# cs2mosa/Heterogeneous-MOE-for-Diffusion-models

Measured on AMD Instinct MI355X. Metric: denoise-steps/sec (fwd+bwd) on 4x32x32 latents, higher is better.
Workload: dtype bf16

## Files before the change

heterogeneous-moe-for-diffusion-models_amd/csrc/common.h:

```cpp
#pragma once
#include <hip/hip_runtime.h>
#include <stdint.h>

#define HDMOE_OK 0
#define HDMOE_EINVAL (-1)
#define HDMOE_EDTYPE (-2)
#define HDMOE_ELAUNCH (-3)

#define HDMOE_F32 0
#define HDMOE_BF16 1
#define HDMOE_F32S 2
#define HDMOE_F16 3

#define HDMOE_MAX_GROUPS 8
#define MP_SILU_DIV 0.596f

typedef __bf16 bf16;
typedef __attribute__((ext_vector_type(8))) __bf16 bf16x8;
typedef __attribute__((ext_vector_type(4))) __bf16 bf16x4;
typedef __attribute__((ext_vector_type(2))) __bf16 bf16x2;
typedef __attribute__((ext_vector_type(16))) float f32x16;
typedef __attribute__((ext_vector_type(4))) float f32x4;

#define DEVI __device__ __forceinline__
// ... 89 lines not shown
}
template <> DEVI void vload<float>(float* f, const float* p) {
  const float4 v = *reinterpret_cast<const float4*>(p);
  f[0] = v.x; f[1] = v.y; f[2] = v.z; f[3] = v.w;
}
template <typename T> DEVI void vstore(T* p, const float* f);
template <> DEVI void vstore<bf16>(bf16* p, const float* f) {
  bf16x8 v;
#pragma unroll
  for (int j = 0; j < 8; ++j) v[j] = (bf16)f[j];
  *reinterpret_cast<bf16x8*>(p) = v;
}
template <> DEVI void vstore<float>(float* p, const float* f) { *reinterpret_cast<float4*>(p) = make_float4(f[0], f[1], f[2], f[3]); }
static inline bool al16(const void* p) { return p == nullptr || ((uintptr_t)p & 15) == 0; }

static inline int hdmoe_launch_status() {
  return hipGetLastError() == hipSuccess ? HDMOE_OK : HDMOE_ELAUNCH;
}
static inline bool hdmoe_first_on_device(unsigned long long& mask) {
  int dev = 0;
  (void)hipGetDevice(&dev);
  const unsigned long long bit = 1ull << (dev & 63);
  if (mask & bit) return false;
  mask |= bit;
  return true;
}
static inline unsigned cdiv(long a, long b) { return (unsigned)((a + b - 1) / b); }

DEVI void philox(uint32_t c0, uint32_t c1, uint32_t k0, uint32_t k1, uint32_t* o) {
  uint32_t c[4] = {c0, c1, 0u, 0u};
// ... 19 lines not shown
```

heterogeneous-moe-for-diffusion-models_amd/csrc/elementwise.hip:

```cpp
#include "common.h"
#include "hdmoe.h"

namespace {

constexpr int TPB = 256;
static inline unsigned grid_for(long n) {
  long b = (n + TPB - 1) / TPB;
  if (b > 2048) b = 2048;
  if (b < 1) b = 1;
  return (unsigned)b;
}
#define GRID_STRIDE(i, n) for (long i = (long)blockIdx.x * blockDim.x + threadIdx.x; i < (n); i += (long)gridDim.x * blockDim.x)

template <typename T>
__global__ void axpby_kernel(T* out, const T* x, const T* y, float a, float b, long n) {
  GRID_STRIDE(i, n) {
    float v = a * to_f(x[i]);
    if (y) v += b * to_f(y[i]);
    out[i] = from_f<T>(v);
  }
}
template <typename T>
__global__ void affine_kernel(T* out, const T* x, float a, float c, long n) {
  GRID_STRIDE(i, n) out[i] = from_f<T>(a * to_f(x[i]) + c);
// ... 582 lines not shown
__global__ void nhwc_to_nchw_guided_kernel(float* out, const T* F, const float* sf, const float* x, const float* sx, float g, int C, long HW,
                                           long n) {
  const float gu = 1.f - g;
  GRID_STRIDE(i, n) {
    long t = i; const long p = t % HW; t /= HW;
    const int c = (int)(t % C); const long b = t / C;
    const long f = (b * HW + p) * C + c;
    float v = gu * to_f(F[n + f]) + g * to_f(F[f]);
    if (sf) v *= sf[b];
    if (x) v += (sx ? sx[b] : 1.f) * x[i];
    out[i] = v;
  }
}

template <typename T, bool TO_IMG>
__global__ void patch_relayout_kernel(T* out, const T* in, int H, int W, int C, int p, int hp, int wp, int order, long n) {
  GRID_STRIDE(i, n) {
    long t = i; const int c = (int)(t % C); t /= C;
    const int x = (int)(t % W); t /= W;
    const int y = (int)(t % H); const long b = t / H;
    const int ph = y / p, ii = y % p, pw = x / p, jj = x % p;
    const int f = order ? c * p * p + ii * p + jj : (ii * p + jj) * C + c;
    const long tk = ((b * hp + ph) * wp + pw) * ((long)C * p * p) + f;
    if (TO_IMG) out[i] = in[tk];
    else out[tk] = in[i];
  }
}

template <typename T, bool TO_IMG>
__global__ void patch_relayout_vec_kernel(T* out, const T* in, int H, int W, int C, int p, int hp, int wp, int order, long nv) {
  constexpr int VW = VT<T>::W;
  const int CV = C / VW;
  GRID_STRIDE(i, nv) {
    long t = i; const int c0 = (int)(t % CV) * VW; t /= CV;
    const int x = (int)(t % W); t /= W;
    const int y = (int)(t % H); const long b = t / H;
    const int ph = y / p, ii = y - ph * p, pw = x / p, jj = x - pw * p;
    const long tb = ((b * hp + ph) * wp + pw) * ((long)C * p * p);
    T* img = (TO_IMG ? out : const_cast<T*>(in)) + i * VW;
    if (order == 0) {
      T* tk = (TO_IMG ? const_cast<T*>(in) : out) + tb + (long)(ii * p + jj) * C + c0;
      if (TO_IMG) *reinterpret_cast<uint4*>(img) = *reinterpret_cast<const uint4*>(tk);
      else *reinterpret_cast<uint4*>(tk) = *reinterpret_cast<const uint4*>(img);
    } else {
      const int pp = p * p;
      T* tk = (TO_IMG ? const_cast<T*>(in) : out) + tb + (long)c0 * pp + ii * p + jj;
      alignas(16) T v[VW];
      if (TO_IMG) {
#pragma unroll
        for (int k = 0; k < VW; ++k) v[k] = tk[(long)k * pp];
        *reinterpret_cast<uint4*>(img) = *reinterpret_cast<const uint4*>(v);
      } else {
        *reinterpret_cast<uint4*>(v) = *reinterpret_cast<const uint4*>(img);
#pragma unroll
        for (int k = 0; k < VW; ++k) tk[(long)k * pp] = v[k];
      }
    }
  }
}

template <typename T>
__global__ void patch_to_tokens_o1_vec_kernel(T* tok, const T* img, int H, int W, int C, int p, int hp, int wp, long nv) {
  constexpr int VW = VT<T>::W;
  const int jv = p / VW;
  GRID_STRIDE(v, nv) {
    long t = v;
    const int j0 = (int)(t % jv) * VW; t /= jv;
    const int ii = (int)(t % p); t /= p;
    const int c = (int)(t % C); t /= C;
    const int pw = (int)(t % wp); t /= wp;
    const int ph = (int)(t % hp); const long b = t / hp;
    const int y = ph * p + ii, x0 = pw * p + j0;
    alignas(16) T vals[VW];
#pragma unroll
    for (int k = 0; k < VW; ++k) vals[k] = (y < H && x0 + k < W) ? img[((b * H + y) * W + x0 + k) * C + c] : from_f<T>(0.f);
    *reinterpret_cast<uint4*>(tok + v * VW) = *reinterpret_cast<const uint4*>(vals);
  }
}

__global__ void fourier_kernel(float* out, const float* x, const float* freqs, const float* phases, int F, long n) {
  GRID_STRIDE(i, n) {
    const long b = i / F; const int f = (int)(i - b * F);
    out[i] = cosf(x[b] * freqs[f] + phases[f]) * 1.41421356237309515f;
  }
}
__global__ void edm_coeffs_kernel(float* coef, const float* sigma, int nsig, float sd, int B) {
  GRID_STRIDE(b, B) {
    const float s = sigma[nsig == 1 ? 0 : b];
    const float q = s * s + sd * sd;
    coef[b] = sd * sd / q;
// ... 690 lines not shown
int hdmoe_nchw_to_nhwc(void* out, const float* x, const float* s, int N, int C, long HW, int dtype, hipStream_t stream) {
  const long n = (long)N * C * HW;
  DT_SWITCH(dtype, L1D(nchw_to_nhwc_kernel<T>, n, (T*)out, x, s, C, HW, n))
}
int hdmoe_nhwc_to_nchw(float* out, const void* F, const float* sf, const float* x, const float* sx, int N, int C, long HW,
                       int dtype, hipStream_t stream) {
  const long n = (long)N * C * HW;
  DT_SWITCH(dtype, L1D(nhwc_to_nchw_kernel<T>, n, out, (const T*)F, sf, x, sx, C, HW, n))
}
int hdmoe_nhwc_to_nchw_guided(float* out, const void* F, const float* sf, const float* x, const float* sx, float g, int N, int C, long HW,
                              int dtype, hipStream_t stream) {
  if (!out || !F || N < 1 || C < 1 || HW < 1 || !(g == g) || g - g != 0.f) return HDMOE_EINVAL;
  const long n = (long)N * C * HW;
  DT_SWITCH(dtype, L1D(nhwc_to_nchw_guided_kernel<T>, n, out, (const T*)F, sf, x, sx, g, C, HW, n))
}
int hdmoe_patch_relayout(void* out, const void* in, int N, int H, int W, int C, int p, int hp, int wp, int order,
                         int to_img, int dtype, hipStream_t stream) {
  if (hp * p < H || wp * p < W) return HDMOE_EINVAL;
  const long n = (long)N * H * W * C;
  if (!to_img && order == 1 && al16(out) && (dtype == HDMOE_BF16 || dtype == HDMOE_F32) && p % (dtype == HDMOE_BF16 ? 8 : 4) == 0) {
    const long nv = (long)N * hp * wp * C * p * p / (dtype == HDMOE_BF16 ? 8 : 4);
    DT_SWITCH(dtype, L1D(patch_to_tokens_o1_vec_kernel<T>, nv, (T*)out, (const T*)in, H, W, C, p, hp, wp, nv))
  }
  if (al16(out) && al16(in) && C % (dtype == HDMOE_BF16 ? 8 : 4) == 0 && (dtype == HDMOE_BF16 || dtype == HDMOE_F32)) {
    const long nv = n / (dtype == HDMOE_BF16 ? 8 : 4);
    if (to_img) { DT_SWITCH(dtype, L1D((patch_relayout_vec_kernel<T, true>), nv, (T*)out, (const T*)in, H, W, C, p, hp, wp, order, nv)) }
    else { DT_SWITCH(dtype, L1D((patch_relayout_vec_kernel<T, false>), nv, (T*)out, (const T*)in, H, W, C, p, hp, wp, order, nv)) }
  }
  if (to_img) { DT_SWITCH(dtype, L1D((patch_relayout_kernel<T, true>), n, (T*)out, (const T*)in, H, W, C, p, hp, wp, order, n)) }
  else { DT_SWITCH(dtype, L1D((patch_relayout_kernel<T, false>), n, (T*)out, (const T*)in, H, W, C, p, hp, wp, order, n)) }
}
int hdmoe_fourier(float* out, const float* x, const float* freqs, const float* phases, int B, int F, hipStream_t stream) {
  const long n = (long)B * F;
  L1D(fourier_kernel, n, out, x, freqs, phases, F, n);
  return hdmoe_launch_status();
}
int hdmoe_edm_coeffs(float* coef, const float* sigma, int nsig, float sigma_data, int B, hipStream_t stream) {
  if (nsig != 1 && nsig != B) return HDMOE_EINVAL;
  L1D(edm_coeffs_kernel, B, coef, sigma, nsig, sigma_data, B);
  return hdmoe_launch_status();
}
int hdmoe_sigmoid_scaling(float* sv, float* su, float* pair, const float* c_noise, float tp, float soft, int B,
                          hipStream_t stream) {
  L1D(sigmoid_scaling_kernel, B, sv, su, pair, c_noise, tp, soft, B);
  return hdmoe_launch_status();
// ... 35 lines not shown
```

heterogeneous-moe-for-diffusion-models_amd/csrc/relayout.hip:

```cpp
#include "common.h"
#include "conv_args.h"
#include "hdmoe.h"

namespace {

constexpr int TPB = 256;
constexpr int RL_MAXV = 8;
constexpr int RL_TILE_MAX = RL_MAXV * TPB * 16;
constexpr int RL_TILE_TARGET = RL_TILE_MAX / 2;
constexpr int RL_PMAX = 64;
constexpr int RL_LDS_BYTES = RL_TILE_MAX + RL_PMAX * 16;
constexpr int RL_GRID = 512;

struct RlArgs {
  void* tok; void* img;
  int H, W, C, p, hp, wp, TW, tpr;
  long ntiles;
};

struct RlTile {
  long img0, tok0;
  int nvec, rowv, RS;
  int ylim, xlimv;
};
template <typename T, int P>
DEVI RlTile rl_tile(const RlArgs& a, long t) {
  constexpr int VW = VT<T>::W;
  const int p = P ? P : a.p;
  const long band = t / a.tpr;
  const int pw0 = (int)(t - band * a.tpr) * a.TW;
  const int tw = a.wp - pw0 < a.TW ? a.wp - pw0 : a.TW;
  const long b = band / a.hp;
// ... 35 lines not shown
  constexpr int VW = VT<T>::W;
  const int p = P ? P : a.p;
  const int jvn = p / VW, KV = a.C * p * jvn;
  const int tl = v / KV, rem = v - tl * KV;
  const int jv = rem % jvn, t2 = rem / jvn;
  const int ii = t2 % p, c = t2 / p;
  return ii * g.RS + (tl * p + jv * VW) * a.C + c;
}

template <typename T, int P, bool TO_IMG>
__global__ __launch_bounds__(TPB) void patch_relayout_tiled_kernel(RlArgs a) {
  constexpr int VW = VT<T>::W;
  __shared__ uint4 lds4[RL_LDS_BYTES / 16];
  T* lds = reinterpret_cast<T*>(lds4);
  uint4 r[RL_MAXV];
  long t = blockIdx.x;
  if (t >= a.ntiles) return;
  RlTile g = rl_tile<T, P>(a, t);
  rl_load<T, P, TO_IMG>(r, a, g);
  while (true) {
#pragma unroll
    for (int k = 0; k < RL_MAXV; ++k) {
      const int v = (int)threadIdx.x + k * TPB;
      if (v < g.nvec) {
        if (TO_IMG) {
          const int o = rl_tok_lds<T, P>(a, g, v);
          alignas(16) T e[VW];
          *reinterpret_cast<uint4*>(e) = r[k];
#pragma unroll
          for (int j = 0; j < VW; ++j) lds[o + j * a.C] = e[j];
        } else {
          const int ii = v / g.rowv, rest = v - ii * g.rowv;
          *reinterpret_cast<uint4*>(lds + ii * g.RS + rest * VW) = r[k];
        }
      }
    }
    __syncthreads();
    const long tn = t + gridDim.x;
    const RlTile gc = g;
    if (tn < a.ntiles) {
      g = rl_tile<T, P>(a, tn);
      rl_load<T, P, TO_IMG>(r, a, g);
    }
#pragma unroll
    for (int k = 0; k < RL_MAXV; ++k) {
      const int v = (int)threadIdx.x + k * TPB;
      if (v < gc.nvec) {
        if (TO_IMG) {
          const int ii = v / gc.rowv, rest = v - ii * gc.rowv;
          if (ii < gc.ylim && rest < gc.xlimv)
            *reinterpret_cast<uint4*>(static_cast<T*>(a.img) + gc.img0 + (long)ii * a.W * a.C + (long)rest * VW) =
                *reinterpret_cast<const uint4*>(lds + ii * gc.RS + rest * VW);
        } else {
          const int o = rl_tok_lds<T, P>(a, gc, v);
          alignas(16) T e[VW];
#pragma unroll
          for (int j = 0; j < VW; ++j) e[j] = lds[o + j * a.C];
          *reinterpret_cast<uint4*>(static_cast<T*>(a.tok) + gc.tok0 + (long)v * VW) = *reinterpret_cast<const uint4*>(e);
        }
      }
    }
    if (tn >= a.ntiles) break;
    t = tn;
    __syncthreads();
  }
}

template <typename T, bool TO_IMG>
int rl_launch(const RlArgs& a, unsigned grid, hipStream_t stream) {
  constexpr int VW = VT<T>::W;
  if (a.p == VW) hipLaunchKernelGGL((patch_relayout_tiled_kernel<T, VW, TO_IMG>), dim3(grid), dim3(TPB), 0, stream, a);
  else if (a.p == 2 * VW) hipLaunchKernelGGL((patch_relayout_tiled_kernel<T, 2 * VW, TO_IMG>), dim3(grid), dim3(TPB), 0, stream, a);
  else if (a.p == 4 * VW) hipLaunchKernelGGL((patch_relayout_tiled_kernel<T, 4 * VW, TO_IMG>), dim3(grid), dim3(TPB), 0, stream, a);
  else hipLaunchKernelGGL((patch_relayout_tiled_kernel<T, 0, TO_IMG>), dim3(grid), dim3(TPB), 0, stream, a);
  return hdmoe_launch_status();
}

constexpr int CR_U = 4;

// ... 56 lines not shown
      vstore<T>(dys + r * L + i, o);
      if (dot) {
        float y[VW];
        vload<T>(y, ys + r * L + i);
#pragma unroll
        for (int k = 0; k < VW; ++k) acc += g[k] * y[k];
      }
    }
  }
  if (dsparse) {
    acc = block_sum(acc, sm);
    if (threadIdx.x == 0 && b >= 0) atomicAdd(&dsparse[(long)b * E + row_expert[r]], acc);
  }
}

}

extern "C" {

int hdmoe_patch_relayout_tiled(void* out, const void* in, int N, int H, int W, int C, int p, int hp, int wp, int order, int to_img,
                               int dtype, hipStream_t stream) {
  if (!out || !in || N < 0 || H < 1 || W < 1 || C < 1 || p < 1 || hp < 1 || wp < 1 || (long)hp * p < H || (long)wp * p < W) return HDMOE_EINVAL;
  if (order != 1 || (dtype != HDMOE_BF16 && dtype != HDMOE_F32)) return 1;
  const int VW = dtype == HDMOE_BF16 ? 8 : 4, esz = dtype == HDMOE_BF16 ? 2 : 4;
  if (p % VW || C % VW || p > RL_PMAX || !al16(out) || !al16(in)) return 1;
  const long tokb = (long)C * p * p * esz;
  if (tokb > RL_TILE_MAX) return 1;
  if (N == 0) return HDMOE_OK;
  RlArgs a;
  a.tok = to_img ? const_cast<void*>(in) : out;
  a.img = to_img ? out : const_cast<void*>(in);
  a.H = H; a.W = W; a.C = C; a.p = p; a.hp = hp; a.wp = wp;
  long TW = RL_TILE_TARGET / tokb;
  if (TW < 1) TW = 1;
  if (TW > wp) TW = wp;
  a.TW = (int)TW;
  a.tpr = (wp + a.TW - 1) / a.TW;
  a.ntiles = (long)N * hp * a.tpr;
  if ((long)N * hp * wp * (tokb / esz) >= (1l << 40)) return 1;
  const unsigned grid = (unsigned)(a.ntiles < RL_GRID ? a.ntiles : RL_GRID);
  hdmoe_count_selection(HDMOE_SEL_RELAYOUT_TILED);
  if (dtype == HDMOE_BF16) return to_img ? rl_launch<bf16, true>(a, grid, stream) : rl_launch<bf16, false>(a, grid, stream);
  return to_img ? rl_launch<float, true>(a, grid, stream) : rl_launch<float, false>(a, grid, stream);
}

int hdmoe_combine_rows_fwd_vec(void* out, const void* ys, const int* inv, const float* row_w, long B, int kcap, long L, int dtype,
                               hipStream_t stream) {
  if (dtype != HDMOE_F32 && dtype != HDMOE_BF16) return HDMOE_EDTYPE;
  if (!out || !ys || !inv || B < 0 || kcap < 1 || L < 1) return HDMOE_EINVAL;
  const int VW = dtype == HDMOE_BF16 ? 8 : 4;
  if (L % VW || !al16(out) || !al16(ys)) return 1;
  if (B == 0) return HDMOE_OK;
  const long nck = cdiv(L, (long)TPB * CR_U * VW);
  if (B * nck >= (1l << 31)) return 1;
  hdmoe_count_selection(HDMOE_SEL_COMBINE_FWD_VEC);
  if (dtype == HDMOE_F32) hipLaunchKernelGGL(combine_rows_fwd_vec_kernel<float>, dim3((unsigned)(B * nck)), dim3(TPB), 0, stream, (float*)out, (const float*)ys, inv, row_w, kcap, L, (unsigned)nck);
  else hipLaunchKernelGGL(combine_rows_fwd_vec_kernel<bf16>, dim3((unsigned)(B * nck)), dim3(TPB), 0, stream, (bf16*)out, (const bf16*)ys, inv, row_w, kcap, L, (unsigned)nck);
  return hdmoe_launch_status();
// ... 18 lines not shown
```

heterogeneous-moe-for-diffusion-models_amd/hdmoe_hip/ops.py:

```python
from __future__ import annotations

import ctypes
import math
from typing import List, Optional, Sequence

import torch

from . import bank as _bank
from ._lib import dtype_code_cast
from ._lib import _int_array, call, dtype_code, lib

Tensor = torch.Tensor


def _c(t: Optional[Tensor]) -> Optional[Tensor]:
    if t is None:
        return None
    return t if t.is_contiguous() else t.contiguous()


def _dt(t: Tensor) -> int:
    return dtype_code(t.dtype)


# ... 651 lines not shown
        ents = [bank.lookup(ws, torch.float32, float(gain), 1.0, True) for ws in layers]
        ok = all(e is not None for e in ents) and len({(e.I, e.Ipad, len(e.params)) for e in ents if e is not None}) == 1
        if ok and all(e.khs == [1] * len(e.params) for e in ents) and (seg is not None or len(ents[0].params) == 1):
            flat = [w for ws in layers for w in ws]
            return list(_MultiLinearFn.apply(x, seg, ents, bank, float(c), *flat))
    outs = [mp_conv(x, ws if seg is not None else ws[0], gain, seg=seg, training=training) for ws in layers]
    return [affine(o, 1.0, c) for o in outs] if c != 0.0 else outs



def _call_or(fast: str, plain: str, *args) -> None:
    if call(fast, *args) == 1:
        call(plain, *args)


class _PatchLinearFn(torch.autograd.Function):

    @staticmethod
    def forward(ctx, x, w, b):
        x = _c(x)
        N, H, W, C = x.shape
        E, p = int(w.shape[0]), int(w.shape[2])
        hp, wp, K = H // p, W // p, C * p * p
        Epad = (E + 15) // 16 * 16
        tok = torch.empty((N, hp, wp, K), dtype=x.dtype, device=x.device)
        _call_or("hdmoe_patch_relayout_tiled", "hdmoe_patch_relayout", tok, x, N, H, W, C, p, hp, wp, 1, 0, _dt(x))
        wf = torch.empty(E * K, dtype=x.dtype, device=x.device)
        wd = torch.empty(K * Epad, dtype=x.dtype, device=x.device) if ctx.needs_input_grad[0] else None
        call("hdmoe_wprep_fwd", [w], None, 1.0, [1], [1], 1, E, K, K, Epad, wf, wf.numel(), wd, 0 if wd is None else wd.numel(), 0, 0, 0, _dt(x))
        y0 = torch.empty((N, hp, wp, E), dtype=x.dtype, device=x.device)
# ... 3 lines not shown
        ctx.save_for_backward(tok, w)
        ctx.wd = wd
        ctx.dims = (N, H, W, C, E, p, hp, wp, K, Epad)
        return y.reshape(N, hp * wp, E)

    @staticmethod
    def backward(ctx, dy):
        tok, w = ctx.saved_tensors
        N, H, W, C, E, p, hp, wp, K, Epad = ctx.dims
        dy = _c(dy).reshape(N, hp, wp, E)
        dt = _dt(dy)
        dx = dw = db = None
        if ctx.needs_input_grad[0]:
            dtok = torch.empty((N, hp, wp, K), dtype=dy.dtype, device=dy.device)
            call("hdmoe_conv_fwd", dy, ctx.wd, dtok, None, 1.0, 0.0, None, 1, ctx.wd.numel(), N, hp, wp, hp, wp, E, E, Epad, K, K, 1, 0, [1], [1], [0], [0], dt)
            dx = torch.empty((N, H, W, C), dtype=dy.dtype, device=dy.device)
            _call_or("hdmoe_patch_relayout_tiled", "hdmoe_patch_relayout", dx, dtok, N, H, W, C, p, hp, wp, 1, 1, dt)
        if ctx.needs_input_grad[1]:
            Gs = [_zeros((1, E, K), torch.float32, dy.device)]
            call("hdmoe_conv_wgrad", tok, dy, Gs, None, 1, N, hp, wp, hp, wp, K, K, E, 1, 0, [1], [1], [0], [0], dt)
            dw = torch.empty_like(w)
            call("hdmoe_wprep_bwd", [w], None, 1.0, Gs, [dw], None, [1], [1], 1, E, K, 0)
        if ctx.needs_input_grad[2]:
            db = torch.zeros(E, dtype=torch.float32, device=dy.device)
            call("hdmoe_colsum", db, dy, N * hp * wp, E, dt)
        return dx, dw, db


class _PatchEmbedFn(torch.autograd.Function):

    @staticmethod
    def forward(ctx, x, w, b):
# ... 17 lines not shown
        x, w = ctx.saved_tensors
        N, H, W, C = x.shape
        E, p = int(w.shape[0]), int(w.shape[2])
        hp, wp = -(-H // p), -(-W // p)
        dy = _c(dy).reshape(N, hp, wp, E)
        dx = dw = db = None
        if ctx.needs_input_grad[0]:
            Ipad = (C + 15) // 16 * 16
            Epad = (E + 15) // 16 * 16
            wf = torch.empty(p * p * E * Ipad, dtype=x.dtype, device=x.device)
            wd = torch.empty(p * p * C * Epad, dtype=x.dtype, device=x.device)
            call("hdmoe_wprep_fwd", [w], None, 1.0, [p], [p], 1, E, C, Ipad, Epad, wf, wf.numel(), wd, wd.numel(), 0, 0, 0, _dt(x))
            tok = torch.empty((N, hp, wp, p * p * C), dtype=x.dtype, device=x.device)
            call("hdmoe_conv_fwd", dy, wd, tok, None, 1.0, 0.0, None, 1, wd.numel(), N, hp, wp, hp, wp, E, E, Epad, p * p * C,
                 p * p * C, 1, 0, [1], [1], [0], [0], _dt(x))
            dx = torch.empty_like(x)
            call("hdmoe_patch_relayout", dx, tok, N, H, W, C, p, hp, wp, 0, 1, _dt(x))
        if ctx.needs_input_grad[1]:
            Gs = [_zeros((p * p, E, C), torch.float32, x.device)]
            call("hdmoe_conv_wgrad", x, dy, Gs, None, 1, N, H, W, hp, wp, C, C, E, p, 0, [p], [p], [0], [0], _dt(x))
            dw = torch.empty_like(w)
            call("hdmoe_wprep_bwd", [w], None, 1.0, Gs, [dw], None, [p], [p], 1, E, C, 0)
        if ctx.needs_input_grad[2]:
            db = torch.zeros(E, dtype=torch.float32, device=x.device)
            call("hdmoe_colsum", db, dy, N * hp * wp, E, _dt(x))
        return dx, dw, db


def patch_embed(x: Tensor, w: Tensor, b: Tensor) -> Tensor:
    p = int(w.shape[2])
    if (x.shape[1] % p == 0 and x.shape[2] % p == 0 and w.shape[2] == w.shape[3] and w.is_contiguous()
            and x.shape[3] % (8 if x.dtype == torch.bfloat16 else 4) == 0 and (x.shape[3] * p * p) % 16 == 0):
        return _PatchLinearFn.apply(x, w, b)
    return _PatchEmbedFn.apply(x, w, b)


class _AxpbyFn(torch.autograd.Function):
    @staticmethod
    def forward(ctx, x, y, a, b):
        x = _c(x); y = _c(y)
        out = torch.empty_like(x)
        call("hdmoe_axpby", out, x, y, a, b, x.numel(), _dt(x))
        ctx.ab = (a, b, y is not None)
        return out

    @staticmethod
    def backward(ctx, g):
        a, b, has_y = ctx.ab
        g = _c(g)
# ... 885 lines not shown

    @staticmethod
    def backward(ctx, g):
        N, H, W, C, p, hp, wp, order = ctx.meta
        g = _c(g)
        dtok = torch.zeros(ctx.tshape, dtype=g.dtype, device=g.device) if (hp * p != H or wp * p != W) else \
            torch.empty(ctx.tshape, dtype=g.dtype, device=g.device)
        _call_or("hdmoe_patch_relayout_tiled", "hdmoe_patch_relayout", dtok, g, N, H, W, C, p, hp, wp, order, 0, _dt(g))
        return dtok, None


def pixel_shuffle_tokens(tok: Tensor, H: int, W: int, C: int, p: int) -> Tensor:
    N = tok.shape[0]
    hp, wp = -(-H // p), -(-W // p)
    return _PatchRelayoutFn.apply(tok, (N, H, W, C, p, hp, wp, 1))


class _PixelNormFn(torch.autograd.Function):
    @staticmethod
    def forward(ctx, x, with_silu, gx_scale=1.0):
        ctx.sx = float(gx_scale)
        x = _c(x)
        C = x.shape[-1]
        xn = torch.empty_like(x)
        h = torch.empty_like(x) if with_silu else None
        call("hdmoe_pixelnorm_fwd", xn, h, x, x.numel() // C, C, _dt(x))
        ctx.save_for_backward(x)
        ctx.with_silu = with_silu
        if with_silu:
            return xn, h
# ... 661 lines not shown
```

heterogeneous-moe-for-diffusion-models_amd/models/model_components.py:

```python
from __future__ import annotations

from typing import List, Optional, Sequence

import torch
import torch.nn as nn

import models.model_internals as m
from hdmoe_hip import ops

Tensor = torch.Tensor


class Scaling_router(nn.Module):

    def __init__(self, emb_dim: Optional[int] = 3, num_experts: Optional[int] = 2, dropout: Optional[float] = 0.2):
        super().__init__()
        self.soft_route = nn.Sequential(
            m.MP_Conv(in_channels=emb_dim, out_channels=emb_dim * 2, kernel=()),
            nn.GroupNorm(1, emb_dim * 2),
            nn.ReLU(),
            m.MP_Conv(in_channels=emb_dim * 2, out_channels=emb_dim * 4, kernel=()),
            nn.GroupNorm(1, emb_dim * 4),
            nn.ReLU(),
            nn.Dropout(dropout),
# ... 424 lines not shown
    h = ops.ln_rag(yn, [b.norm2.weight for b in blocks], [b.norm2.bias for b in blocks], rag, b0.norm2.eps)
    h = ops.mp_silu(lin([b.linear2 for b in blocks], h, b0.gain_s))
    h = lin([b.linear3 for b in blocks], h, b0.gain_s, res=y, alpha=(1.0 - bal) / n, beta=bal / n, res_grad_raw=True)
    if b0.skip_proj is not None:
        return lin([b.skip_proj for b in blocks], res_main, b0.gain_s, res=h, alpha=(1.0 - bal) / n, beta=bal / n)
    return ops.mp_sum(res_main, h, bal)


def vit_expert_bank_forward(experts: Sequence["Vit_expert"], x: Tensor, time_emb: Optional[Tensor], text_emb: Optional[Tensor],
                            seg: Tensor) -> Tensor:
    e0 = experts[0]
    tr = e0.training
    R, H, W, C = x.shape
    ps = [e.patch.kernel_size[0] for e in experts]
    rag = ops.RagLayout(seg, [(-(-H // p)) * (-(-W // p)) for p in ps], R)
    pes = [ops.patch_embed(xe, e.patch.weight, e.patch.bias) for xe, e in zip(ops.fanout(x, len(experts)), experts)]
    tok = ops.rag_pack(pes, [e.pos_emb for e in experts], rag)
    t = time_emb
    if text_emb is not None:
        tx = text_emb
        if e0.map_txt is not None:
            tx = ops.mp_conv(tx, [e.map_txt.weights for e in experts], seg=seg, training=tr)
        t = ops.mp_sum(t, tx, e0.emb_balance)
    nb = len(e0.diffit)
    timed = t is not None and e0.diffit[0].TMSA.time_dependent
    tps = ts = None
    if timed and 3 * nb <= 16 and len({b.gain_t for b in e0.diffit}) == 1:
        layers = [[getattr(e.diffit[i].TMSA, nm).weights for e in experts] for i in range(nb) for nm in ("q_time", "k_time", "v_time")]
        tps = ops.multi_linear(t, layers, e0.diffit[0].gain_t, seg=seg, training=tr)
    elif timed:
        ts = list(ops.fanout(t, 3 * nb))
    for i in range(nb):
        tok = vit_block_bank_forward([e.diffit[i] for e in experts], tok, t if ts is None else ts[3 * i:3 * i + 3], rag,
                                     None if tps is None else tps[3 * i:3 * i + 3])
    tok = ops.ln_rag(tok, [e.norm.weight for e in experts], [e.norm.bias for e in experts], rag, e0.norm.eps)
    outs = []
    for e, p, part in zip(experts, ps, ops.rag_unpack(tok, rag)):
        outs.append(ops.pixel_shuffle_tokens(e.unpatch_proj._fwd(part), H, W, C, p))
    return ops.rag_select(outs, rag)
```

include/hdmoe.h:

```cpp
#ifndef HDMOE_H
#define HDMOE_H
#ifdef __cplusplus
extern "C" {
#endif

#ifndef HDMOE_OK
#define HDMOE_OK 0
#define HDMOE_EINVAL (-1)
#define HDMOE_EDTYPE (-2)
#define HDMOE_ELAUNCH (-3)
#define HDMOE_F32 0
#define HDMOE_BF16 1
#define HDMOE_F16 3
#define HDMOE_F32S 2
#define HDMOE_MAX_GROUPS 8
#endif

typedef void* hdmoe_stream_t;
#ifdef __HIPCC__
#define HS hipStream_t
#else
#define HS hdmoe_stream_t
#endif

// ... 54 lines not shown
  HDMOE_SEL_BWD7_16_OT1 = 7,
  HDMOE_SEL_BWD7_16_OT2 = 8,
  HDMOE_SEL_BWD6 = 9,
  HDMOE_SEL_BWD6S = 10,
  HDMOE_SEL_WGRAD6_DIRECT = 11,
  HDMOE_SEL_WGRAD6_DEFER = 12,
  HDMOE_SEL_BLK6 = 13,
  HDMOE_SEL_WGRAD8_C11 = 14,
  HDMOE_SEL_WGRAD8_C12 = 15,
  HDMOE_SEL_WGRAD8_C21 = 16,
  HDMOE_SEL_WGRAD8_C22 = 17,
  HDMOE_SEL_PW_BWD = 18,
  HDMOE_SEL_RELAYOUT_TILED = 19,
  HDMOE_SEL_COMBINE_FWD_VEC = 20,
  HDMOE_SEL_COMBINE_BWD_VEC = 21,
  HDMOE_SEL_COUNT = 22
};
int hdmoe_kernel_selections(long long* counts, int n, int reset);

int hdmoe_wbank_desc_bytes(void);
int hdmoe_wbank_prep(const void* descs, const int* rows, int nrows, int mutate, HS stream);
int hdmoe_wbank_bwd(const void* descs, const int* rows, int nrows, HS stream);

int hdmoe_axpby(void* out, const void* x, const void* y, float a, float b, long n, int dtype, HS stream);
int hdmoe_sum_n(void* out, const void* const* srcs, const float* src_scale, int n, long nelem, int dtype, HS stream);
int hdmoe_affine(void* out, const void* x, float a, float c, long n, int dtype, HS stream);
int hdmoe_mul(void* out, const void* x, const void* y, long n, int dtype, HS stream);
int hdmoe_sched_pick(float* sigma, const double* t, const int* idx, int off, HS stream);
int hdmoe_idx_advance(int* idx, HS stream);
int hdmoe_heun_euler(float* xn, const float* xh, const float* den, const double* t, const int* idx, long n,
                     const float* x0, const float* noise, const float* mask, HS stream);
// ... 48 lines not shown
int hdmoe_gate_mix_fwd(void* out, float* gate, const void* logits, const void* U, const void* A, long rows, int C,
                       int dtype, HS stream);
int hdmoe_gate_mix_bwd(void* dU, void* dA, void* dlogits, const void* dout, const float* dgate, const float* gate,
                       const void* U, const void* A, long rows, int C, int dtype, HS stream);
int hdmoe_softmax_rows_fwd(float* out, const float* x, long rows, int C, float scale, HS stream);
int hdmoe_softmax_rows_bwd(float* dx, const float* dy, const float* y, long rows, int C, float scale, HS stream);
int hdmoe_nchw_to_nhwc(void* out, const float* x, const float* s, int N, int C, long HW, int dtype, HS stream);
int hdmoe_nhwc_to_nchw(float* out, const void* F, const float* sf, const float* x, const float* sx, int N, int C,
                       long HW, int dtype, HS stream);
int hdmoe_nhwc_to_nchw_guided(float* out, const void* F, const float* sf, const float* x, const float* sx, float g, int N,
                              int C, long HW, int dtype, HS stream);
int hdmoe_patch_relayout(void* out, const void* in, int N, int H, int W, int C, int p, int hp, int wp, int order,
                         int to_img, int dtype, HS stream);
int hdmoe_patch_relayout_tiled(void* out, const void* in, int N, int H, int W, int C, int p, int hp, int wp, int order,
                               int to_img, int dtype, HS stream);
int hdmoe_fourier(float* out, const float* x, const float* freqs, const float* phases, int B, int F, HS stream);
int hdmoe_edm_coeffs(float* coef, const float* sigma, int nsig, float sigma_data, int B, HS stream);
int hdmoe_sigmoid_scaling(float* sv, float* su, float* pair, const float* c_noise, float tp, float soft, int B, HS stream);
int hdmoe_adaln_fwd(float* out, const float* x, const float* cond, long B, int F, HS stream);
int hdmoe_adaln_bwd(float* dx, float* dcond, const float* g, const float* x, const float* cond, long B, int F, HS stream);
int hdmoe_take_col_pos_fwd(float* out, const float* w, long B, int E, int e, HS stream);
int hdmoe_take_col_pos_bwd(float* dw, const float* g, const float* w, long B, int E, int e, HS stream);
int hdmoe_dropout(void* out, const void* x, unsigned long long seed, const unsigned long long* seed_dev, float p, long n, int dtype,
                  HS stream);
int hdmoe_randn(float* out, unsigned long long seed, const unsigned long long* seed_dev, float scale, long n, HS stream);
int hdmoe_seed_advance(unsigned long long* seed_dev, HS stream);

int hdmoe_pixelnorm_fwd(void* xn, void* h, const void* x, long rows, int C, int dtype, HS stream);
int hdmoe_pixelnorm_bwd(void* dx, const void* dxn, const void* dh, const void* x, long rows, int C, float sx, int dtype, HS stream);
int hdmoe_groupnorm_fwd(void* y, float* mean, float* rstd, const void* x, const float* gamma, const float* beta, int N,
// ... 129 lines not shown
```

Measured before the change: 79.57.

## Restrict patch relayout to each expert's row window in MoE ViT paths

Adds row-window variants of the patch relayout kernels that process only the rows routed to a given expert group (from device-side segment offsets) and zero or skip the others. The unpatch path now writes each expert's tokens directly into one shared output, replacing per-expert full-image shuffles followed by rag_select. Patch-embed backward likewise writes each expert's dx slice straight into one shared buffer instead of building full per-expert gradients through fanout. The aim is to cut redundant relayout traffic and the extra select/fanout kernels and allocations, at the cost of more complex indexing and reliance on the segment layout being correct.

Result: no change. 80.13 (median of 6 runs) (+0.7%).

```diff
diff --git a/heterogeneous-moe-for-diffusion-models_amd/csrc/common.h b/heterogeneous-moe-for-diffusion-models_amd/csrc/common.h
--- a/heterogeneous-moe-for-diffusion-models_amd/csrc/common.h
+++ b/heterogeneous-moe-for-diffusion-models_amd/csrc/common.h
@@ -127,6 +127,14 @@
 template <> DEVI void vstore<float>(float* p, const float* f) { *reinterpret_cast<float4*>(p) = make_float4(f[0], f[1], f[2], f[3]); }
 static inline bool al16(const void* p) { return p == nullptr || ((uintptr_t)p & 15) == 0; }
 
+struct RowWin { const int* seg2; const int* tail; int fill; };
+enum { ROW_SKIP = 0, ROW_OWN = 1, ROW_ZERO = 2 };
+DEVI int row_win(const RowWin& w, long row) {
+  if (!w.seg2) return ROW_OWN;
+  if (row >= w.seg2[0] && row < w.seg2[1]) return ROW_OWN;
+  return (w.fill || (w.tail && row >= *w.tail)) ? ROW_ZERO : ROW_SKIP;
+}
+
 static inline int hdmoe_launch_status() {
   return hipGetLastError() == hipSuccess ? HDMOE_OK : HDMOE_ELAUNCH;
 }
diff --git a/heterogeneous-moe-for-diffusion-models_amd/csrc/elementwise.hip b/heterogeneous-moe-for-diffusion-models_amd/csrc/elementwise.hip
--- a/heterogeneous-moe-for-diffusion-models_amd/csrc/elementwise.hip
+++ b/heterogeneous-moe-for-diffusion-models_amd/csrc/elementwise.hip
@@ -1,4 +1,5 @@
 #include "common.h"
+#include "conv_args.h"
 #include "hdmoe.h"
 
 namespace {
@@ -620,33 +621,40 @@
 }
 
 template <typename T, bool TO_IMG>
-__global__ void patch_relayout_kernel(T* out, const T* in, int H, int W, int C, int p, int hp, int wp, int order, long n) {
+__global__ void patch_relayout_kernel(T* out, const T* in, int H, int W, int C, int p, int hp, int wp, int order, long n, RowWin win) {
   GRID_STRIDE(i, n) {
     long t = i; const int c = (int)(t % C); t /= C;
     const int x = (int)(t % W); t /= W;
     const int y = (int)(t % H); const long b = t / H;
+    const int own = row_win(win, b);
+    if (own == ROW_SKIP) continue;
     const int ph = y / p, ii = y % p, pw = x / p, jj = x % p;
     const int f = order ? c * p * p + ii * p + jj : (ii * p + jj) * C + c;
     const long tk = ((b * hp + ph) * wp + pw) * ((long)C * p * p) + f;
-    if (TO_IMG) out[i] = in[tk];
+    if (own == ROW_ZERO) out[TO_IMG ? i : tk] = from_f<T>(0.f);
+    else if (TO_IMG) out[i] = in[tk];
     else out[tk] = in[i];
   }
 }
 
 template <typename T, bool TO_IMG>
-__global__ void patch_relayout_vec_kernel(T* out, const T* in, int H, int W, int C, int p, int hp, int wp, int order, long nv) {
+__global__ void patch_relayout_vec_kernel(T* out, const T* in, int H, int W, int C, int p, int hp, int wp, int order, long nv, RowWin win) {
   constexpr int VW = VT<T>::W;
   const int CV = C / VW;
   GRID_STRIDE(i, nv) {
     long t = i; const int c0 = (int)(t % CV) * VW; t /= CV;
     const int x = (int)(t % W); t /= W;
     const int y = (int)(t % H); const long b = t / H;
+    const int own = row_win(win, b);
+    if (own == ROW_SKIP) continue;
     const int ph = y / p, ii = y - ph * p, pw = x / p, jj = x - pw * p;
     const long tb = ((b * hp + ph) * wp + pw) * ((long)C * p * p);
     T* img = (TO_IMG ? out : const_cast<T*>(in)) + i * VW;
+    if (own == ROW_ZERO && TO_IMG) { *reinterpret_cast<uint4*>(img) = make_uint4(0, 0, 0, 0); continue; }
     if (order == 0) {
       T* tk = (TO_IMG ? const_cast<T*>(in) : out) + tb + (long)(ii * p + jj) * C + c0;
-      if (TO_IMG) *reinterpret_cast<uint4*>(img) = *reinterpret_cast<const uint4*>(tk);
+      if (own == ROW_ZERO) *reinterpret_cast<uint4*>(tk) = make_uint4(0, 0, 0, 0);
+      else if (TO_IMG) *reinterpret_cast<uint4*>(img) = *reinterpret_cast<const uint4*>(tk);
       else *reinterpret_cast<uint4*>(tk) = *reinterpret_cast<const uint4*>(img);
     } else {
       const int pp = p * p;
@@ -657,7 +665,7 @@
         for (int k = 0; k < VW; ++k) v[k] = tk[(long)k * pp];
         *reinterpret_cast<uint4*>(img) = *reinterpret_cast<const uint4*>(v);
       } else {
-        *reinterpret_cast<uint4*>(v) = *reinterpret_cast<const uint4*>(img);
+        *reinterpret_cast<uint4*>(v) = own == ROW_ZERO ? make_uint4(0, 0, 0, 0) : *reinterpret_cast<const uint4*>(img);
 #pragma unroll
         for (int k = 0; k < VW; ++k) tk[(long)k * pp] = v[k];
       }
@@ -666,7 +674,7 @@
 }
 
 template <typename T>
-__global__ void patch_to_tokens_o1_vec_kernel(T* tok, const T* img, int H, int W, int C, int p, int hp, int wp, long nv) {
+__global__ void patch_to_tokens_o1_vec_kernel(T* tok, const T* img, int H, int W, int C, int p, int hp, int wp, long nv, RowWin win) {
   constexpr int VW = VT<T>::W;
   const int jv = p / VW;
   GRID_STRIDE(v, nv) {
@@ -676,10 +684,12 @@
     const int c = (int)(t % C); t /= C;
     const int pw = (int)(t % wp); t /= wp;
     const int ph = (int)(t % hp); const long b = t / hp;
+    const int own = row_win(win, b);
+    if (own == ROW_SKIP) continue;
     const int y = ph * p + ii, x0 = pw * p + j0;
     alignas(16) T vals[VW];
 #pragma unroll
-    for (int k = 0; k < VW; ++k) vals[k] = (y < H && x0 + k < W) ? img[((b * H + y) * W + x0 + k) * C + c] : from_f<T>(0.f);
+    for (int k = 0; k < VW; ++k) vals[k] = (own == ROW_OWN && y < H && x0 + k < W) ? img[((b * H + y) * W + x0 + k) * C + c] : from_f<T>(0.f);
     *reinterpret_cast<uint4*>(tok + v * VW) = *reinterpret_cast<const uint4*>(vals);
   }
 }
@@ -1400,21 +1410,31 @@
   const long n = (long)N * C * HW;
   DT_SWITCH(dtype, L1D(nhwc_to_nchw_guided_kernel<T>, n, out, (const T*)F, sf, x, sx, g, C, HW, n))
 }
-int hdmoe_patch_relayout(void* out, const void* in, int N, int H, int W, int C, int p, int hp, int wp, int order,
-                         int to_img, int dtype, hipStream_t stream) {
+static int patch_relayout_launch(void* out, const void* in, int N, int H, int W, int C, int p, int hp, int wp, int order,
+                                 int to_img, int dtype, RowWin win, hipStream_t stream) {
   if (hp * p < H || wp * p < W) return HDMOE_EINVAL;
   const long n = (long)N * H * W * C;
   if (!to_img && order == 1 && al16(out) && (dtype == HDMOE_BF16 || dtype == HDMOE_F32) && p % (dtype == HDMOE_BF16 ? 8 : 4) == 0) {
     const long nv = (long)N * hp * wp * C * p * p / (dtype == HDMOE_BF16 ? 8 : 4);
-    DT_SWITCH(dtype, L1D(patch_to_tokens_o1_vec_kernel<T>, nv, (T*)out, (const T*)in, H, W, C, p, hp, wp, nv))
+    DT_SWITCH(dtype, L1D(patch_to_tokens_o1_vec_kernel<T>, nv, (T*)out, (const T*)in, H, W, C, p, hp, wp, nv, win))
   }
   if (al16(out) && al16(in) && C % (dtype == HDMOE_BF16 ? 8 : 4) == 0 && (dtype == HDMOE_BF16 || dtype == HDMOE_F32)) {
     const long nv = n / (dtype == HDMOE_BF16 ? 8 : 4);
-    if (to_img) { DT_SWITCH(dtype, L1D((patch_relayout_vec_kernel<T, true>), nv, (T*)out, (const T*)in, H, W, C, p, hp, wp, order, nv)) }
-    else { DT_SWITCH(dtype, L1D((patch_relayout_vec_kernel<T, false>), nv, (T*)out, (const T*)in, H, W, C, p, hp, wp, order, nv)) }
-  }
-  if (to_img) { DT_SWITCH(dtype, L1D((patch_relayout_kernel<T, true>), n, (T*)out, (const T*)in, H, W, C, p, hp, wp, order, n)) }
-  else { DT_SWITCH(dtype, L1D((patch_relayout_kernel<T, false>), n, (T*)out, (const T*)in, H, W, C, p, hp, wp, order, n)) }
+    if (to_img) { DT_SWITCH(dtype, L1D((patch_relayout_vec_kernel<T, true>), nv, (T*)out, (const T*)in, H, W, C, p, hp, wp, order, nv, win)) }
+    else { DT_SWITCH(dtype, L1D((patch_relayout_vec_kernel<T, false>), nv, (T*)out, (const T*)in, H, W, C, p, hp, wp, order, nv, win)) }
+  }
+  if (to_img) { DT_SWITCH(dtype, L1D((patch_relayout_kernel<T, true>), n, (T*)out, (const T*)in, H, W, C, p, hp, wp, order, n, win)) }
+  else { DT_SWITCH(dtype, L1D((patch_relayout_kernel<T, false>), n, (T*)out, (const T*)in, H, W, C, p, hp, wp, order, n, win)) }
+}
+int hdmoe_patch_relayout(void* out, const void* in, int N, int H, int W, int C, int p, int hp, int wp, int order,
+                         int to_img, int dtype, hipStream_t stream) {
+  return patch_relayout_launch(out, in, N, H, W, C, p, hp, wp, order, to_img, dtype, RowWin{nullptr, nullptr, 0}, stream);
+}
+int hdmoe_patch_relayout_win(void* out, const void* in, int N, int H, int W, int C, int p, int hp, int wp, int order,
+                             int to_img, int dtype, const int* seg2, const int* tail, int fill, hipStream_t stream) {
+  if (!out || !in || !seg2 || N < 0) return HDMOE_EINVAL;
+  hdmoe_count_selection(HDMOE_SEL_RELAYOUT_WIN);
+  return patch_relayout_launch(out, in, N, H, W, C, p, hp, wp, order, to_img, dtype, RowWin{seg2, tail, fill}, stream);
 }
 int hdmoe_fourier(float* out, const float* x, const float* freqs, const float* phases, int B, int F, hipStream_t stream) {
   const long n = (long)B * F;
diff --git a/heterogeneous-moe-for-diffusion-models_amd/csrc/relayout.hip b/heterogeneous-moe-for-diffusion-models_amd/csrc/relayout.hip
--- a/heterogeneous-moe-for-diffusion-models_amd/csrc/relayout.hip
+++ b/heterogeneous-moe-for-diffusion-models_amd/csrc/relayout.hip
@@ -16,6 +16,9 @@
   void* tok; void* img;
   int H, W, C, p, hp, wp, TW, tpr;
   long ntiles;
+  RowWin win;
+  int N;
+  long out_row16;
 };
 
 struct RlTile {
@@ -81,8 +84,15 @@
   __shared__ uint4 lds4[RL_LDS_BYTES / 16];
   T* lds = reinterpret_cast<T*>(lds4);
   uint4 r[RL_MAXV];
-  long t = blockIdx.x;
-  if (t >= a.ntiles) return;
+  long t = blockIdx.x, tend = a.ntiles;
+  int lo = 0, hi = a.N;
+  if (a.win.seg2) {
+    lo = min(max(a.win.seg2[0], 0), a.N);
+    hi = min(max(a.win.seg2[1], lo), a.N);
+    const long tpi = (long)a.hp * a.tpr;
+    t += lo * tpi; tend = hi * tpi;
+  }
+  if (t < tend) {
   RlTile g = rl_tile<T, P>(a, t);
   rl_load<T, P, TO_IMG>(r, a, g);
   while (true) {
@@ -105,7 +115,7 @@
     __syncthreads();
     const long tn = t + gridDim.x;
     const RlTile gc = g;
-    if (tn < a.ntiles) {
+    if (tn < tend) {
       g = rl_tile<T, P>(a, tn);
       rl_load<T, P, TO_IMG>(r, a, g);
     }
@@ -127,9 +137,18 @@
         }
       }
     }
-    if (tn >= a.ntiles) break;
+    if (tn >= tend) break;
     t = tn;
     __syncthreads();
+  }
+  }
+  if (a.win.seg2 && (a.win.fill || a.win.tail)) {
+    uint4* o = static_cast<uint4*>(TO_IMG ? a.img : a.tok);
+    const long z0 = a.win.fill ? lo : 0;
+    const long z1 = a.win.fill ? hi : min(max((long)*a.win.tail, (long)hi), (long)a.N);
+    const long nlo = z0 * a.out_row16, nhi = (a.N - z1) * a.out_row16;
+    for (long i = (long)blockIdx.x * TPB + threadIdx.x; i < nlo + nhi; i += (long)gridDim.x * TPB)
+      o[i < nlo ? i : z1 * a.out_row16 + (i - nlo)] = make_uint4(0, 0, 0, 0);
   }
 }
 
@@ -216,12 +235,8 @@
   }
 }
 
-}
-
-extern "C" {
-
-int hdmoe_patch_relayout_tiled(void* out, const void* in, int N, int H, int W, int C, int p, int hp, int wp, int order, int to_img,
-                               int dtype, hipStream_t stream) {
+int rl_entry(void* out, const void* in, int N, int H, int W, int C, int p, int hp, int wp, int order, int to_img, int dtype, RowWin win,
+             int sel, hipStream_t stream) {
   if (!out || !in || N < 0 || H < 1 || W < 1 || C < 1 || p < 1 || hp < 1 || wp < 1 || (long)hp * p < H || (long)wp * p < W) return HDMOE_EINVAL;
   if (order != 1 || (dtype != HDMOE_BF16 && dtype != HDMOE_F32)) return 1;
   const int VW = dtype == HDMOE_BF16 ? 8 : 4, esz = dtype == HDMOE_BF16 ? 2 : 4;
@@ -240,10 +255,25 @@
   a.tpr = (wp + a.TW - 1) / a.TW;
   a.ntiles = (long)N * hp * a.tpr;
   if ((long)N * hp * wp * (tokb / esz) >= (1l << 40)) return 1;
+  a.win = win; a.N = N;
+  a.out_row16 = (to_img ? (long)H * W * C : (long)hp * wp * (tokb / esz)) * esz / 16;
   const unsigned grid = (unsigned)(a.ntiles < RL_GRID ? a.ntiles : RL_GRID);
-  hdmoe_count_selection(HDMOE_SEL_RELAYOUT_TILED);
+  hdmoe_count_selection(sel);
   if (dtype == HDMOE_BF16) return to_img ? rl_launch<bf16, true>(a, grid, stream) : rl_launch<bf16, false>(a, grid, stream);
   return to_img ? rl_launch<float, true>(a, grid, stream) : rl_launch<float, false>(a, grid, stream);
+}
+}
+
+extern "C" {
+
+int hdmoe_patch_relayout_tiled(void* out, const void* in, int N, int H, int W, int C, int p, int hp, int wp, int order, int to_img,
+                               int dtype, hipStream_t stream) {
+  return rl_entry(out, in, N, H, W, C, p, hp, wp, order, to_img, dtype, RowWin{nullptr, nullptr, 0}, HDMOE_SEL_RELAYOUT_TILED, stream);
+}
+int hdmoe_patch_relayout_tiled_win(void* out, const void* in, int N, int H, int W, int C, int p, int hp, int wp, int order, int to_img,
+                                   int dtype, const int* seg2, const int* tail, int fill, hipStream_t stream) {
+  if (!seg2) return HDMOE_EINVAL;
+  return rl_entry(out, in, N, H, W, C, p, hp, wp, order, to_img, dtype, RowWin{seg2, tail, fill}, HDMOE_SEL_RELAYOUT_TILED_WIN, stream);
 }
 
 int hdmoe_combine_rows_fwd_vec(void* out, const void* ys, const int* inv, const float* row_w, long B, int kcap, long L, int dtype,
diff --git a/heterogeneous-moe-for-diffusion-models_amd/hdmoe_hip/ops.py b/heterogeneous-moe-for-diffusion-models_amd/hdmoe_hip/ops.py
--- a/heterogeneous-moe-for-diffusion-models_amd/hdmoe_hip/ops.py
+++ b/heterogeneous-moe-for-diffusion-models_amd/hdmoe_hip/ops.py
@@ -689,6 +689,20 @@
         call(plain, *args)
 
 
+_empty = torch.empty
+
+
+def _relayout(out, src, N, H, W, C, p, hp, wp, order, to_img, dt, win=None, fill=0) -> None:
+    if win is None:
+        if order != 1 or call("hdmoe_patch_relayout_tiled", out, src, N, H, W, C, p, hp, wp, order, to_img, dt) == 1:
+            call("hdmoe_patch_relayout", out, src, N, H, W, C, p, hp, wp, order, to_img, dt)
+        return
+    seg, g, G = win
+    seg2, tail = seg[g:g + 2], (seg[G:G + 1] if g == G - 1 and not fill else None)
+    if call("hdmoe_patch_relayout_tiled_win", out, src, N, H, W, C, p, hp, wp, order, to_img, dt, seg2, tail, fill) == 1:
+        call("hdmoe_patch_relayout_win", out, src, N, H, W, C, p, hp, wp, order, to_img, dt, seg2, tail, fill)
+
+
 class _PatchLinearFn(torch.autograd.Function):
 
     @staticmethod
@@ -722,8 +736,9 @@
         if ctx.needs_input_grad[0]:
             dtok = torch.empty((N, hp, wp, K), dtype=dy.dtype, device=dy.device)
             call("hdmoe_conv_fwd", dy, ctx.wd, dtok, None, 1.0, 0.0, None, 1, ctx.wd.numel(), N, hp, wp, hp, wp, E, E, Epad, K, K, 1, 0, [1], [1], [0], [0], dt)
-            dx = torch.empty((N, H, W, C), dtype=dy.dtype, device=dy.device)
-            _call_or("hdmoe_patch_relayout_tiled", "hdmoe_patch_relayout", dx, dtok, N, H, W, C, p, hp, wp, 1, 1, dt)
+            win = getattr(ctx, "win", None)
+            dx = torch.empty((N, H, W, C), dtype=dy.dtype, device=dy.device) if win is None else win[0]
+            _relayout(dx, dtok, N, H, W, C, p, hp, wp, 1, 1, dt, None if win is None else win[1:])
         if ctx.needs_input_grad[1]:
             Gs = [_zeros((1, E, K), torch.float32, dy.device)]
             call("hdmoe_conv_wgrad", tok, dy, Gs, None, 1, N, hp, wp, hp, wp, K, K, E, 1, 0, [1], [1], [0], [0], dt)
@@ -771,8 +786,9 @@
             tok = torch.empty((N, hp, wp, p * p * C), dtype=x.dtype, device=x.device)
             call("hdmoe_conv_fwd", dy, wd, tok, None, 1.0, 0.0, None, 1, wd.numel(), N, hp, wp, hp, wp, E, E, Epad, p * p * C,
                  p * p * C, 1, 0, [1], [1], [0], [0], _dt(x))
-            dx = torch.empty_like(x)
-            call("hdmoe_patch_relayout", dx, tok, N, H, W, C, p, hp, wp, 0, 1, _dt(x))
+            win = getattr(ctx, "win", None)
+            dx = torch.empty_like(x) if win is None else win[0]
+            _relayout(dx, tok, N, H, W, C, p, hp, wp, 0, 1, _dt(x), None if win is None else win[1:])
         if ctx.needs_input_grad[1]:
             Gs = [_zeros((p * p, E, C), torch.float32, x.device)]
             call("hdmoe_conv_wgrad", x, dy, Gs, None, 1, N, H, W, hp, wp, C, C, E, p, 0, [p], [p], [0], [0], _dt(x))
@@ -784,12 +800,58 @@
         return dx, dw, db
 
 
-def patch_embed(x: Tensor, w: Tensor, b: Tensor) -> Tensor:
+def _patch_fn(x: Tensor, w: Tensor):
     p = int(w.shape[2])
     if (x.shape[1] % p == 0 and x.shape[2] % p == 0 and w.shape[2] == w.shape[3] and w.is_contiguous()
             and x.shape[3] % (8 if x.dtype == torch.bfloat16 else 4) == 0 and (x.shape[3] * p * p) % 16 == 0):
-        return _PatchLinearFn.apply(x, w, b)
-    return _PatchEmbedFn.apply(x, w, b)
+        return _PatchLinearFn
+    return _PatchEmbedFn
+
+
+def patch_embed(x: Tensor, w: Tensor, b: Tensor) -> Tensor:
+    return _patch_fn(x, w).apply(x, w, b)
+
+
+class _SubCtx:
+
+    def __init__(self, needs_input_grad):
+        self.needs_input_grad, self.saved_tensors, self.win = needs_input_grad, (), None
+
+    def save_for_backward(self, *ts):
+        self.saved_tensors = ts
+
+
+class _PatchEmbedBankFn(torch.autograd.Function):
+
+    @staticmethod
+    def forward(ctx, x, rag, *tensors):
+        G = rag.G
+        x = _c(x)
+        nig = ctx.needs_input_grad
+        subs, ys = [], []
+        for g in range(G):
+            fn, sub = _patch_fn(x, tensors[g]), _SubCtx((nig[0], nig[2 + g], nig[2 + G + g]))
+            ys.append(fn.forward(sub, x, tensors[g], tensors[G + g]))
+            subs.append((fn, sub))
+        ctx.subs, ctx.rag, ctx.xmeta = subs, rag, (x.shape, x.dtype, x.device)
+        return tuple(ys)
+
+    @staticmethod
+    def backward(ctx, *dys):
+        rag, G = ctx.rag, ctx.rag.G
+        shape, dtype, device = ctx.xmeta
+        dx = _empty(shape, dtype=dtype, device=device) if ctx.needs_input_grad[0] else None
+        dws, dbs = [], []
+        for g, (fn, sub) in enumerate(ctx.subs):
+            sub.win = (dx, rag.seg, g, G)
+            _, dw, db = fn.backward(sub, dys[g])
+            dws.append(dw)
+            dbs.append(db)
+        return (dx, None, *dws, *dbs)
+
+
+def patch_embed_bank(x: Tensor, ws: Sequence[Tensor], bs: Sequence[Tensor], rag: "RagLayout"):
+    return _PatchEmbedBankFn.apply(x, rag, *ws, *bs)
 
 
 class _AxpbyFn(torch.autograd.Function):
@@ -1705,6 +1767,39 @@
     N = tok.shape[0]
     hp, wp = -(-H // p), -(-W // p)
     return _PatchRelayoutFn.apply(tok, (N, H, W, C, p, hp, wp, 1))
+
+
+class _UnpatchBankFn(torch.autograd.Function):
+
+    @staticmethod
+    def forward(ctx, rag, meta, *toks):
+        H, W, C, ps = meta
+        G, R = rag.G, rag.R
+        toks = [_c(t) for t in toks]
+        out = _empty((R, H, W, C), dtype=toks[0].dtype, device=toks[0].device)
+        for g, (t, p) in enumerate(zip(toks, ps)):
+            _relayout(out, t, R, H, W, C, p, -(-H // p), -(-W // p), 1, 1, _dt(t), (rag.seg, g, G))
+        ctx.rag, ctx.meta, ctx.tshapes = rag, meta, [t.shape for t in toks]
+        return out
+
+    @staticmethod
+    def backward(ctx, gout):
+        H, W, C, ps = ctx.meta
+        rag = ctx.rag
+        gout = _c(gout)
+        vw = 8 if gout.dtype == torch.bfloat16 else 4
+        dtoks = []
+        for g, (shape, p) in enumerate(zip(ctx.tshapes, ps)):
+            hp, wp = -(-H // p), -(-W // p)
+            padded = (hp * p != H or wp * p != W) and (p % vw != 0 or gout.data_ptr() % 16 != 0)
+            d = torch.zeros(shape, dtype=gout.dtype, device=gout.device) if padded else _empty(shape, dtype=gout.dtype, device=gout.device)
+            _relayout(d, gout, rag.R, H, W, C, p, hp, wp, 1, 0, _dt(gout), (rag.seg, g, rag.G), fill=1)
+            dtoks.append(d)
+        return (None, None, *dtoks)
+
+
+def unpatch_bank(toks: Sequence[Tensor], rag: "RagLayout", H: int, W: int, C: int, ps: Sequence[int]) -> Tensor:
+    return _UnpatchBankFn.apply(rag, (int(H), int(W), int(C), tuple(int(p) for p in ps)), *toks)
 
 
 class _PixelNormFn(torch.autograd.Function):
diff --git a/heterogeneous-moe-for-diffusion-models_amd/models/model_components.py b/heterogeneous-moe-for-diffusion-models_amd/models/model_components.py
--- a/heterogeneous-moe-for-diffusion-models_amd/models/model_components.py
+++ b/heterogeneous-moe-for-diffusion-models_amd/models/model_components.py
@@ -462,7 +462,7 @@
     R, H, W, C = x.shape
     ps = [e.patch.kernel_size[0] for e in experts]
     rag = ops.RagLayout(seg, [(-(-H // p)) * (-(-W // p)) for p in ps], R)
-    pes = [ops.patch_embed(xe, e.patch.weight, e.patch.bias) for xe, e in zip(ops.fanout(x, len(experts)), experts)]
+    pes = ops.patch_embed_bank(x, [e.patch.weight for e in experts], [e.patch.bias for e in experts], rag)
     tok = ops.rag_pack(pes, [e.pos_emb for e in experts], rag)
     t = time_emb
     if text_emb is not None:
@@ -482,7 +482,5 @@
         tok = vit_block_bank_forward([e.diffit[i] for e in experts], tok, t if ts is None else ts[3 * i:3 * i + 3], rag,
                                      None if tps is None else tps[3 * i:3 * i + 3])
     tok = ops.ln_rag(tok, [e.norm.weight for e in experts], [e.norm.bias for e in experts], rag, e0.norm.eps)
-    outs = []
-    for e, p, part in zip(experts, ps, ops.rag_unpack(tok, rag)):
-        outs.append(ops.pixel_shuffle_tokens(e.unpatch_proj._fwd(part), H, W, C, p))
-    return ops.rag_select(outs, rag)
+    toks = [e.unpatch_proj._fwd(part) for e, part in zip(experts, ops.rag_unpack(tok, rag))]
+    return ops.unpatch_bank(toks, rag, H, W, C, ps)
diff --git a/include/hdmoe.h b/include/hdmoe.h
--- a/include/hdmoe.h
+++ b/include/hdmoe.h
@@ -92,7 +92,9 @@
   HDMOE_SEL_RELAYOUT_TILED = 19,
   HDMOE_SEL_COMBINE_FWD_VEC = 20,
   HDMOE_SEL_COMBINE_BWD_VEC = 21,
-  HDMOE_SEL_COUNT = 22
+  HDMOE_SEL_RELAYOUT_TILED_WIN = 22,
+  HDMOE_SEL_RELAYOUT_WIN = 23,
+  HDMOE_SEL_COUNT = 24
 };
 int hdmoe_kernel_selections(long long* counts, int n, int reset);
 
@@ -171,6 +173,10 @@
                          int to_img, int dtype, HS stream);
 int hdmoe_patch_relayout_tiled(void* out, const void* in, int N, int H, int W, int C, int p, int hp, int wp, int order,
                                int to_img, int dtype, HS stream);
+int hdmoe_patch_relayout_win(void* out, const void* in, int N, int H, int W, int C, int p, int hp, int wp, int order,
+                             int to_img, int dtype, const int* seg2, const int* tail, int fill, HS stream);
+int hdmoe_patch_relayout_tiled_win(void* out, const void* in, int N, int H, int W, int C, int p, int hp, int wp, int order,
+                                   int to_img, int dtype, const int* seg2, const int* tail, int fill, HS stream);
 int hdmoe_fourier(float* out, const float* x, const float* freqs, const float* phases, int B, int F, HS stream);
 int hdmoe_edm_coeffs(float* coef, const float* sigma, int nsig, float sigma_data, int B, HS stream);
 int hdmoe_sigmoid_scaling(float* sv, float* su, float* pair, const float* c_noise, float tp, float soft, int B, HS stream);
```
